# andreicuceu/vega

Measured on AMD Instinct MI355X. Metric: model+chi2 evals/sec (Lya auto+cross), higher is better.
Workload: dtype f64

## Files before the change

### vega_amd/csrc/vegamx.hip

```cpp
#include "vmx_device.h"
#include "vmx_fit.h"
#include "vmx_ensemble.h"
#include "vmx_nested.h"
#include "vmx_smc.h"

#include <atomic>
#include <cmath>
#include <chrono>
#include <thread>
#include <algorithm>
#include <cstdio>
#include <cstdlib>
#include <cstring>
#include <map>
#include <mutex>
#include <queue>
#include <utility>
#include <string>
#include <vector>

#ifndef VMX_MAX_LANES
#define VMX_MAX_LANES 2
#endif

// ... 624 lines not shown
    std::vector<hipEvent_t> ev_join;
    bool finalized = false;
    std::vector<vmx_engine*> lanes;
    int n_lanes = 1;
    int64_t lane_calls = 0;
    hipStream_t last_stream = nullptr;
    const int32_t* call_mock = nullptr;
    FitWorkspace* fitws = nullptr;
    EnsWorkspace* ensws = nullptr;
    NsWorkspace* nsws = nullptr;
    SmcWorkspace* smcws = nullptr;
    hipEvent_t lane_wait = nullptr;

    int nk = 0, nkp = 0, n_mu = 0;
    int n_rows = 0, n_extra = 0, mu_lo = 0, mu_hi = 0;
    DevBuf<double> node_w, mu_img, mu_img_w;
    std::vector<int32_t> rule_slot; std::vector<double> rule_lo, rule_hi;
    DevBuf<int32_t> d_rule_slot; DevBuf<double> d_rule_lo, d_rule_hi;
    double k_node_max = 0.0; bool mu_nodes_on = true;
    DevBuf<double> k, pklin, delta2, mu, sq1mmu2, lnmu, wl, gk, gk_mom, fv_x, fv_f, xtab;
    std::vector<int32_t> const_slots;
    std::vector<int32_t> const_slots2;
    DevBuf<int32_t> d_const_slots, d_const_slots2, d_xtab_pipe, d_xtab_partner;
    DevBuf<double> xtab_k;
    std::vector<int32_t> xi_static_taps, xi_static_bins;
    DevBuf<int32_t> d_xi_static_taps, d_xi_static_bins;
    DevBuf<unsigned long long> gemm_trace;
    size_t gemm_trace_blocks = 0;
    DevBuf<unsigned long long> pk_trace;
    size_t pk_trace_blocks = 0;
    std::vector<int32_t> w_groups;
    DevBuf<int32_t> d_w_groups;
    bool no_pk_w = false;
    std::vector<Tab2Group> tab2_groups;
    DevBuf<double> xtab_key;
    int n_xtab = 0;
    int const_hint = 0;
    int fv_n = 0;
    struct GkSpec { double rp, rt, mock_rp, mock_rt; };
    std::vector<GkSpec> gk_tables;
    std::vector<double> h_k, h_mu;

    int n_coef = 0, ncp = 0, n_knots = 0;
    DevBuf<double> op;
    bool op_set[VMX_MAX_ELL] = {false, false, false, false};
    bool extrapolate = false;
    double x0[VMX_MAX_ELL] = {0}, h[VMX_MAX_ELL] = {0};

    std::vector<PipeDev> pipes;
    std::vector<double> h_r, h_mu_c, h_z, h_relz, h_lnrelz, h_lnrelz2, h_growth;
    DevBuf<double> cr, cmu, crp, crt, cz, crelz, clnrelz, clnrelz2, cgrowth;
    DevBuf<PipeDev> d_pipes;
    std::vector<PkGroup> pk_groups;
    DevBuf<PkGroup> d_pk_groups;
    std::vector<int32_t> pk_members, pk_poly, pk_static;
    DevBuf<int32_t> d_pk_members, d_pk_poly, d_pk_static, d_pipe_active;
    DevBuf<double> poly_coef, poly_bins;
    int64_t poly_bins_total = 0;
    int n_active = 0;
    bool poly_dirty = true;

    std::vector<ItemHost*> items;
    std::vector<MetalHost*> metals;
    DevBuf<ItemDev> d_items;
    DevBuf<MetalDev> d_metals;
    std::vector<double> h_bb, h_odd, h_odd_op;
// ... 1082 lines not shown
int vmx_add_prior(vmx_engine* e, int32_t slot, double mean, double sigma)
{
    REQUIRE(e && !e->finalized && slot >= 0 && sigma != 0.0, "vmx_add_prior");
    e->prior_slot.push_back(slot); e->prior_mean.push_back(mean); e->prior_sigma.push_back(sigma);
    return 0;
}

static int poly_basis_build(vmx_engine* e);
static int xi_sum_plan(vmx_engine* e);

int vmx_finalize(vmx_engine* e, int32_t n_params, int32_t max_batch)
{
    REQUIRE(e && !e->finalized, "vmx_finalize");
    REQUIRE(n_params > 0 && max_batch > 0, "n_params / max_batch");
    REQUIRE(e->nk > 0 && !e->pipes.empty() && !e->items.empty(), "template, pipelines and items are required");
    REQUIRE(e->items.size() <= 16, "at most 16 correlation items");
    REQUIRE(e->pipes.size() * sizeof(PipeDev) <= 48 * 1024, "too many pipelines for the prologue's descriptor stage");
    for (int i = 0; i < VMX_MAX_ELL; ++i) REQUIRE(e->op_set[i], "all four FFTLog operators are required");
    HIP_OK(hipSetDevice(e->device));
    const int Bm = max_batch;
    e->n_params = n_params; e->max_batch = Bm;
    e->slab_rows = Bm > 1024 ? Bm : 1024;
    e->fact_slab_rows = std::max(1024, std::min(4 * Bm, 8192));
    if (getenv("VMX_NO_GRAPH")) e->use_graphs = false;
    if (getenv("VMX_TRACE_HOST")) e->trace_host = true;
    {
        int cus = 256;
        if (hipDeviceGetAttribute(&cus, hipDeviceAttributeMultiprocessorCount, e->device) != hipSuccess || cus <= 0) { (void)hipGetLastError(); cus = 256; }
        e->quad_blocks = 2 * cus;
    }
    if (getenv("VMX_NO_TAB2")) e->no_tab2 = true;
    if (getenv("VMX_NO_CINV_TAPE")) e->no_cinv_tape = true;
    if (getenv("VMX_NO_PK_W")) e->no_pk_w = true;
    if (getenv("VMX_NO_HOST_REDUCE")) e->no_host_reduce = true;
    if (getenv("VMX_NO_XI_LEAN")) e->xi_lean = false;
    if (getenv("VMX_NO_XI_SUMS")) e->xi_sums = false;

    auto slot_ok = [&](int s) { return s < n_params; };
    for (auto& p : e->pipes) {
        const vmx_pipe_desc& d = p.d;
        const int slots[] = {d.tracer[0].bias_slot, d.tracer[0].bias_eta_slot, d.tracer[0].beta_slot,
                             d.tracer[0].vd_sigma_slot, d.tracer[0].alpha_slot, d.tracer[1].bias_slot,
                             d.tracer[1].bias_eta_slot, d.tracer[1].beta_slot, d.tracer[1].vd_sigma_slot,
                             d.tracer[1].alpha_slot, d.growth_rate_slot, d.bias_gamma_slot, d.bias_prim_slot,
                             d.lambda_uv_slot, d.bias_gamma_e_slot, d.lambda_heii_slot, d.bias_hcd_slot,
                             d.beta_hcd_slot, d.l0_hcd_slot, d.sigma_nl_par_slot, d.sigma_nl_per_slot,
                             d.exp_par_slot, d.exp_per_slot, d.scale_slot[0], d.scale_slot[1], d.drp_slot,
                             d.croom_slot[0], d.croom_slot[1], d.mock_los_slot};
        for (int s : slots) REQUIRE(slot_ok(s), "pipeline slot exceeds n_params");
        for (int i = 0; i < 6; ++i) REQUIRE(slot_ok(d.arinyo_slot[i]), "arinyo slot exceeds n_params");
        for (int i = 0; i < d.n_smooth; ++i)
            REQUIRE(d.smooth_par_slot[i] >= 0 && d.smooth_per_slot[i] >= 0 && slot_ok(d.smooth_par_slot[i]) &&
                    slot_ok(d.smooth_per_slot[i]), "smoothing slot");
        for (int q = 0; q < 2; ++q) {
            const vmx_tracer& t = d.tracer[q];
            const int have = (t.bias_slot >= 0) + (t.bias_eta_slot >= 0) + (t.beta_slot >= 0);
            REQUIRE(have >= 2, "each tracer needs two of (bias, bias_eta, beta)");
            REQUIRE(t.evol_kind == VMX_EVOL_CROOM ? (d.croom_slot[0] >= 0 && d.croom_slot[1] >= 0) : t.alpha_slot >= 0,
                    "bias-evolution slot");
            REQUIRE(d.vd_kind == VMX_VD_NONE || !t.discrete || t.vd_sigma_slot >= 0, "velocity dispersion slot");
        }
        REQUIRE(!d.uvb || (d.bias_gamma_slot >= 0 && d.bias_prim_slot >= 0 && d.lambda_uv_slot >= 0), "UVB slots");
        REQUIRE(!d.heii || (d.bias_gamma_e_slot >= 0 && d.bias_prim_slot >= 0 && d.lambda_heii_slot >= 0), "HeII slots");
        REQUIRE(d.hcd_model == VMX_HCD_NONE || (d.bias_hcd_slot >= 0 && d.beta_hcd_slot >= 0), "HCD slots");
        REQUIRE(d.hcd_model != VMX_HCD_ROGERS || d.l0_hcd_slot >= 0, "L0_hcd slot");
        REQUIRE(d.hcd_model != VMX_HCD_FVOIGT || e->fv_n >= 2, "model-hcd = fvoigt needs vmx_set_fvoigt_table");
// ... 774 lines not shown
            hipLaunchKernelGGL(k_pk_poly, dim3(B, (int)e->pk_poly.size()), dim3(256), 0, e->stream, D, e->d_pk_poly.p, B);
        int tm = tab_mode;
        int n_other = n_groups;
        if (tab_mode >= 2 && e->n_xtab > 0) {
            n_other = n_groups - e->n_xtab;
            const size_t sh1 = std::max<size_t>(2048, (size_t)2 * e->n_mu + 4 * e->n_extra + 256 + 16) * sizeof(double);
            if (sh1 > 64 * 1024) {
                static std::mutex mu;
                static size_t allowed[64] = {};
                std::lock_guard<std::mutex> lock(mu);
                size_t& a = allowed[e->device & 63];
                if (sh1 > a) {
                    HIP_OK(hipFuncSetAttribute((const void*)k_pk_tab2<64, 4, 2>, hipFuncAttributeMaxDynamicSharedMemorySize, (int)sh1));
                    HIP_OK(hipFuncSetAttribute((const void*)k_pk_tab2<64, 4, 1>, hipFuncAttributeMaxDynamicSharedMemorySize, (int)sh1));
                    HIP_OK(hipFuncSetAttribute((const void*)k_pk_tab2<16, 16, 1>, hipFuncAttributeMaxDynamicSharedMemorySize, (int)sh1));
                    a = sh1;
                }
            }
#ifdef VMX_EXP_PRO_TRACE
            D.pk_trace = nullptr;
            if (false) {
#else
            if (getenv("VMX_PK_TRACE")) {
#endif
                e->pk_trace_blocks = (size_t)B * ((e->nk + 7) / 8) * e->tab2_groups.size();
                if (!e->pk_trace.p && e->pk_trace.alloc(4 * (size_t)e->max_batch * ((e->nk + 7) / 8) * e->tab2_groups.size(), true)) return -2;
                D.pk_trace = e->pk_trace.p;
            }
            for (size_t first = 0; first < e->tab2_groups.size(); first += VMX_TAB2_GROUPS) {
                Tab2Args A{};
                const int n = (int)std::min<size_t>(VMX_TAB2_GROUPS, e->tab2_groups.size() - first);
                for (int q = 0; q < n; ++q) A.g[q] = e->tab2_groups[first + q];
                if ((int64_t)B * e->n_xtab >= 24) {
                    if (B >= 64)
                        hipLaunchKernelGGL((k_pk_tab2<64, 4, 2>), dim3((B + 1) / 2, n, (e->nk + 63) / 64), dim3(256), std::max(sh1, (size_t)4096 * sizeof(double)), e->stream, D, A, B);
                    else
                        hipLaunchKernelGGL((k_pk_tab2<64, 4, 1>), dim3(B, n, (e->nk + 63) / 64), dim3(256), sh1, e->stream, D, A, B);
                } else
                    hipLaunchKernelGGL((k_pk_tab2<16, 16, 1>), dim3(B, n, (e->nk + 15) / 16), dim3(256), sh1, e->stream, D, A, B);
            }
        }
        const int n_w = ((int64_t)B * (int)e->w_groups.size() >= 24 && !e->no_pk_w) ? (int)e->w_groups.size() : 0;
        if (n_w > 0) {
            n_other -= n_w;
            tm |= 32;
            const size_t shw = std::max<size_t>((size_t)2 * 6 * 256, (size_t)2 * e->n_mu + 4 * e->n_extra + 16) * sizeof(double);
            if (B >= 64)
                hipLaunchKernelGGL((k_pk_w<2>), dim3((B + 1) / 2, n_w, (e->nk + 63) / 64), dim3(256), shw, e->stream, D, e->d_pk_groups.p, e->d_pk_members.p, e->d_w_groups.p, B);
            else
                hipLaunchKernelGGL((k_pk_w<1>), dim3(B, n_w, (e->nk + 63) / 64), dim3(256), shw, e->stream, D, e->d_pk_groups.p, e->d_pk_members.p, e->d_w_groups.p, B);
        }
        if (n_other == 0) {}
        else {
            bool generic = false;
            for (auto& g : e->pk_groups) if (g.variant == PKV_GENERIC) generic = true;
            const PkGroup* gp = e->d_pk_groups.p;
            const int32_t* mp = e->d_pk_members.p;
#define VMX_LAUNCH_PK(KT, MS)                                                                                        \
            do {                                                                                                     \
                const dim3 grid(B, n_groups, (e->nk + (KT) - 1) / (KT));                                             \
                if (generic) hipLaunchKernelGGL((k_pk_multipoles<KT, MS, 1, true>), grid, dim3(256), shmem, e->stream, D, gp, mp, tm, B, mu_tab_off);   \
                else hipLaunchKernelGGL((k_pk_multipoles<KT, MS, 1, false>), grid, dim3(256), shmem, e->stream, D, gp, mp, tm, B, mu_tab_off);         \
            } while (0)
            if ((int64_t)B * n_groups >= 24) VMX_LAUNCH_PK(64, 4);
            else if ((int64_t)B * n_groups >= 4) VMX_LAUNCH_PK(16, 16);
            else {
                shmem = ((size_t)e->n_rows + 2048 + (size_t)8 * e->n_rows) * sizeof(double);
// ... 2048 lines not shown
```

### vega_amd/csrc/vmx_device.h

```cpp
#pragma once
#include <hip/hip_runtime.h>
#include <stdint.h>
#include "../../include/vegamx.h"
#include "vmx_plan.h"

#define VMX_NS 40
#define VMX_PAD 32
#define VMX_MAX_BB 32
#define VMX_MAX_METALS 64
#define VMX_MAX_QUAD_COEF 64
#define VMX_MAX_GROUP 8
#define VMX_MAX_MARG 16

enum {
    S_BIAS1 = 0, S_BB1, S_BIAS2, S_BB2,
    S_UV_BG, S_UV_BP, S_UV_LAM, S_HE_BG, S_HE_LAM,
    S_HCD_B, S_HCD_BB, S_HCD_L0,
    S_GA, S_GB, S_EA, S_EB,
    S_AQ1, S_AQ2, S_AKV, S_AAV, S_ABV, S_AKP,
    S_VD1, S_VD2,
    S_AP, S_AT, S_DRP, S_EV1A, S_EV1B, S_EV2A, S_EV2B,
    S_RAD_S, S_RAD_A, S_RAD_L, S_RAD_D, S_RAD_IL, S_RAD_ID,
    S_NO_RULE
};

static inline int vmx_pad(int n) { return (n + VMX_PAD - 1) / VMX_PAD * VMX_PAD; }

struct PipeDev {
    vmx_pipe_desc d;
    int32_t n;
    int32_t n_pad;
    int64_t coord_off;
    int64_t xi_off;
    double rp_absmin, rp_absmax, rt_min, rt_max;
    int32_t col;
    int32_t poly_basis;
// ... 184 lines not shown
        const double sp = t[d.smooth_par_slot[i]], st = t[d.smooth_per_slot[i]];
        ga += d.smooth_weight[i] * sp * sp; gb += d.smooth_weight[i] * st * st;
    }
    if (d.vd_kind == VMX_VD_GAUSS)
#pragma unroll
        for (int q = 0; q < 2; ++q)
            if (d.tracer[q].discrete) { const double sg = t[d.tracer[q].vd_sigma_slot]; ga += 0.25 * sg * sg; }
}

#define XTAB_ROWS 8
__device__ __forceinline__ double vmx_log(double x);
__device__ void xtab_body(const EngineDev& D, int xtab, int bx, int by, int rows_per_block, const double* t0);

template <bool BYVAL>
__device__ __forceinline__ void prologue_body(const EngineDev& D, int B)
{
    const double* src_all = BYVAL ? (const double*)__builtin_amdgcn_kernarg_segment_ptr() : D.theta_host ? D.theta_host : D.theta;
    if (D.xtab_block0 > 0 && (int)blockIdx.x >= D.xtab_block0) {
        const int rows_per_block = XTAB_ROWS * (256 / PRO_T);
        const int nbx = (D.nkp + PRO_T - 1) / PRO_T, nby = (D.n_rows + rows_per_block - 1) / rows_per_block;
        const int q = (int)blockIdx.x - D.xtab_block0;
        xtab_body(D, q / (nbx * nby), q % nbx, (q / nbx) % nby, rows_per_block, src_all);
        return;
    }
#ifdef VMX_EXP_PRO_TRACE
#define PRO_STAMP(I) do { if (threadIdx.x == 0 && D.pk_trace) D.pk_trace[8 * blockIdx.x + (I)] = wall_clock64(); } while (0)
#else
#define PRO_STAMP(I) do {} while (0)
#endif
    PRO_STAMP(0);
    const int n_chunk = (B + PRO_T - 1) / PRO_T;
    const int slot = (int)blockIdx.x / n_chunk, b_first = ((int)blockIdx.x % n_chunk) * PRO_T;
    const int b = b_first + (int)threadIdx.x;
    if (blockIdx.x == 0 && threadIdx.x == 0) { D.k_live[0] = 0; D.k_live[1] = 0; }
    const bool half_b = slot >= D.n_pipe && slot < 2 * D.n_pipe, walker_slot = slot == 2 * D.n_pipe;
    const int p = min(half_b ? slot - D.n_pipe : slot, D.n_pipe - 1);
    const VMX_CAS PipeDev& P = *(const VMX_CAS PipeDev*)(D.pipes + p);
    extern __shared__ double s_dyn[];
    const int n_cs = D.n_const_slots, n_ru = D.n_rule;
    double* s_c0 = s_dyn;
    double* s_cs = s_c0 + n_cs;
    double* s_ru = s_cs + n_cs;
    double* s_theta = s_ru + 3 * n_ru;
    const int t_ld = D.n_params | 1;
    const int rows = min(B, b_first + PRO_T) - b_first;
    {
        if (BYVAL || D.src_host) {
            const int count = rows * D.n_params;
            const double* src = src_all + (size_t)b_first * D.n_params;
            for (int i0 = threadIdx.x; i0 < count; i0 += 4 * PRO_T) {
                double v[4];
#pragma unroll
                for (int u = 0; u < 4; ++u) { const int i = i0 + u * PRO_T; v[u] = i < count ? src[i] : 0.0; }
#pragma unroll
                for (int u = 0; u < 4; ++u) { const int i = i0 + u * PRO_T; if (i < count) s_theta[(i / D.n_params) * t_ld + i % D.n_params] = v[u]; }
            }
        } else {
            const int nd = 2 * D.n_params;
            const char* src = (const char*)(src_all + (size_t)b_first * D.n_params);
            for (int c0 = 0; c0 < nd; c0 += PRO_T)
                if (c0 + (int)threadIdx.x < nd)
                    for (int r = 0; r < rows; ++r)
                        __builtin_amdgcn_global_load_lds((const __attribute__((address_space(1))) void*)(src + ((size_t)r * nd + c0 + threadIdx.x) * 4),
                                                         (__attribute__((address_space(3))) void*)((char*)(s_theta + r * t_ld) + c0 * 4), 4, 0, 0);
        }
        if (walker_slot)
            for (int i = threadIdx.x; i < n_cs; i += PRO_T) { const int q = D.const_slots[i]; s_cs[i] = (double)q; s_c0[i] = src_all[q]; }
// ... 874 lines not shown
        s_red[(half * 4 + 2) * 256 + threadIdx.x] = (39.375 * m[2] - 33.75 * m[1] + 3.375 * m[0]) * inv_nmu;
        s_red[(half * 4 + 3) * 256 + threadIdx.x] = (187.6875 * m[3] - 255.9375 * m[2] + 85.3125 * m[1] - 4.0625 * m[0]) * inv_nmu;
    }
    __syncthreads();
    if (bad && valid && walker_ok) atomicOr(&D.status[b], VMX_STATUS_ARINYO);

    if (lt < KT && valid && walker_ok) {
        double damp = 1.0;
        if (d.damping_scale > 0.0) damp = exp(-d.damping_scale * d.damping_scale * pow(k, (double)d.damping_power) / 2.0);
        const size_t ncols = (size_t)B * D.n_active;
        for (int half = 0; half < (T.paired ? 2 : 1); ++half) {
            const int pipe = half ? pp : p;
            const int kind = D.pipes[pipe].d.pk_lin_kind;
            const double pk = damp * ((D.pk_direct && kind == VMX_PKLIN_SMOOTH) ? D.pk_direct[(size_t)b * D.nkp + i]
                                                                                 : D.pklin[(size_t)kind * D.nkp + i]);
            const size_t col = (size_t)D.pipes[pipe].col * B + b;
            for (int e = 0; e < D.n_ell; ++e) {
                double sum = 0.0;
                for (int qq = 0; qq < MS; ++qq) sum += s_red[(half * 4 + e) * 256 + (wb * MS + qq) * KT + kk];
                D.pl[((size_t)e * ncols + col) * D.nkp + i] = pk * sum;
            }
        }
    }
}

struct Tab2Group { int32_t pipe, partner, xtab, cross, kind_s, kind_q, col_s, col_q, uvb, heii, lya1, lya2, damping_power, pad;
                   double damping_scale; };
#define VMX_TAB2_GROUPS 8
struct Tab2Args { Tab2Group g[VMX_TAB2_GROUPS]; };

#ifndef VMX_TAB2_PF
#define VMX_TAB2_PF 4
#endif
template <int KT, int MS, int NW, bool CROSS, int MODE = 0>
__device__ __forceinline__ void pk_tab2_body(const EngineDev& D, const Tab2Group& G, int B)
{
    extern __shared__ double smem[];
    constexpr int NT = KT * MS;
    double* s_red = smem;
    v2d* s_mu24 = (v2d*)smem;
    v4d* s_node = (v4d*)(smem + 2 * D.n_mu);
    const int p = G.pipe, pp = G.partner, xt = G.xtab;
    constexpr bool cross = CROSS;
    const int tile = blockIdx.z;
    const unsigned long long t_start = D.pk_trace ? wall_clock64() : 0ull;
    const int kk = threadIdx.x % KT;
    const int ms = (KT == 64) ? __builtin_amdgcn_readfirstlane(threadIdx.x / KT) : (int)(threadIdx.x / KT);
    const int i = tile * KT + kk;
    const bool valid = i < D.nk;
    const int ic = valid ? i : D.nk - 1;
    const int n_mu = D.n_mu;
    const double inv_nmu = 1.0 / (double)n_mu;
    {
        const unsigned total = (2u * (unsigned)n_mu + 4u * (unsigned)D.n_extra) * 8u;
        const char* img = (const char*)D.mu_img;
        const unsigned wave_off = (threadIdx.x >> 6) * 1024u, lane_off = (threadIdx.x & 63) * 16u;
        for (unsigned c = 0; c < total; c += (unsigned)NT * 16u) {
            const unsigned off = c + wave_off;
            if (off + lane_off < total)
                __builtin_amdgcn_global_load_lds((const __attribute__((address_space(1))) void*)(img + off + lane_off),
                                                 (__attribute__((address_space(3))) void*)((char*)smem + off), 16, 0, 0);
        }
    }
    const double* kx = D.xtab_k + (size_t)xt * 4 * D.nkp + ic;
    const double e_max = kx[3 * D.nkp];
    const double bad_flag = kx[2 * D.nkp];
    const double k = D.k[ic], k2 = k * k;
    bool ok[NW];
    double raw[NW][14];
#pragma unroll
    for (int w = 0; w < NW; ++w) {
        int b = blockIdx.x * NW + w;
        ok[w] = b < B;
        if (!ok[w]) b = B - 1;
        const double* sc = D.scal + ((size_t)b * D.n_pipe + p) * VMX_NS;
        raw[w][0] = sc[S_BIAS1]; raw[w][1] = sc[S_BIAS2]; raw[w][2] = sc[S_BB1]; raw[w][3] = sc[S_BB2];
        raw[w][4] = sc[S_HCD_B]; raw[w][5] = sc[S_HCD_BB]; raw[w][6] = sc[S_HCD_L0]; raw[w][7] = sc[S_VD2]; raw[w][8] = sc[S_NO_RULE];
        raw[w][9] = G.uvb ? sc[S_UV_LAM] : 0.0; raw[w][10] = G.uvb ? sc[S_UV_BG] : 0.0; raw[w][11] = (G.uvb || G.heii) ? sc[S_UV_BP] : 0.0;
        raw[w][12] = G.heii ? sc[S_HE_LAM] : 0.0; raw[w][13] = G.heii ? sc[S_HE_BG] : 0.0;
    }
    double* s_x = smem + 2 * (size_t)n_mu + 4 * (size_t)D.n_extra;
    int* s_vote = (int*)(s_x + 2 * NW * KT);
    if (G.uvb || G.heii) {
#pragma unroll
        for (int role = 0; role < 2 * NW; ++role) {
            if (role % MS != ms) continue;
            const int term = role / NW, wsel = role % NW;
            const double lam = term ? raw[wsel][12] : raw[wsel][9], bg = term ? raw[wsel][13] : raw[wsel][10], bp = raw[wsel][11];
            double v = 0.0;
            if (term ? G.heii : G.uvb) { const double x = k * lam; const double W = atan(x) / x; v = bg * W / (1.0 + bp * W); }
            s_x[(size_t)role * KT + kk] = v;
        }
    }
    {
        const unsigned long long live_v = __ballot(!(e_max < VMX_PK_DEAD));
        const unsigned long long rule_v = __ballot(k <= D.k_node_max || e_max < VMX_PK_NEGLIGIBLE), all_v = __ballot(true);
        if ((threadIdx.x & 63) == 0) {
            s_vote[2 * (threadIdx.x >> 6)] = live_v != 0ull;
            s_vote[2 * (threadIdx.x >> 6) + 1] = rule_v == all_v;
        }
    }
    asm volatile("s_waitcnt vmcnt(0)" ::: "memory");
    __syncthreads();
    bool live_block = false, rule_ok = true;
#pragma unroll
    for (int wv = 0; wv < NT / 64; ++wv) { live_block = live_block || s_vote[2 * wv] != 0; rule_ok = rule_ok && s_vote[2 * wv + 1] != 0; }
    if (!live_block) {
        if (threadIdx.x >= KT || !valid) return;
        const size_t ncols = (size_t)B * D.n_active;
        for (int w = 0; w < NW; ++w) {
            const int b = blockIdx.x * NW + w;
            if (b >= B) continue;
            for (int half = 0; half < 2; ++half)
                for (int e = 0; e < D.n_ell; ++e)
                    D.pl[((size_t)e * ncols + (size_t)(half ? G.col_q : G.col_s) * B + b) * D.nkp + i] = 0.0;
        }
        return;
    }
    const double dmu = (double)MS * inv_nmu;
    const bool bad = bad_flag != 0.0;
    double c01[NW], c11[NW], c02[NW], c12[NW], hb[NW], hbb[NW], fk[NW], Fq[NW], k2vd2[NW];
    bool in_box = true;
#pragma unroll
    for (int w = 0; w < NW; ++w) {
        c01[w] = raw[w][0]; c02[w] = raw[w][1]; c11[w] = raw[w][2]; c12[w] = raw[w][3];
        hb[w] = raw[w][4]; hbb[w] = raw[w][5];
        fk[w] = -raw[w][6] * k;
        Fq[w] = vmx_exp(fk[w] * dmu);
        k2vd2[w] = k2 * raw[w][7];
        const bool inside = raw[w][8] == 0.0;
        in_box = in_box && inside;
        if (MODE == 1) ok[w] = ok[w] && inside;
        if (MODE == 2) ok[w] = ok[w] && !inside;
    }
    if (MODE == 1) in_box = true;
    if (MODE == 2) in_box = false;
    if (threadIdx.x == 0) atomicMax(D.k_live, min((tile + 1) * KT, D.nk));
    const bool node_mode = D.n_extra > 0 && in_box && rule_ok;
    if (node_mode && threadIdx.x == 0) atomicMax(D.k_live + 1, min((tile + 1) * KT, D.nk));
    const int lo_end = node_mode ? D.mu_lo : n_mu, hi_beg = node_mode ? n_mu - D.mu_hi : n_mu;
    if (G.uvb || G.heii) {
#pragma unroll
        for (int w = 0; w < NW; ++w) {
            double add = 0.0;
// ... 81 lines not shown
                for (int w = 0; w < NW; ++w) F[w] = vmx_exp(fk[w] * nd.x);                                            \
                VMX_TAB2_NODE(nd.y, nd.z, true, g, h)                                                                 \
            }
            int jj = ms;
            for (int it = 0; it < steps / VMX_TAB2_PF; ++it, jj += VMX_TAB2_PF * MS) {
#pragma unroll
                for (int u = 0; u < VMX_TAB2_PF; ++u) VMX_TAB2_XSTEP(gw[u], hw[u], jj + u * MS)
            }
#pragma unroll
            for (int u = 0; u < VMX_TAB2_PF - 1; ++u)
                if (u < steps % VMX_TAB2_PF) VMX_TAB2_XSTEP(gw[u], hw[u], jj + u * MS)
#undef VMX_TAB2_XSTEP
        }
#undef VMX_TAB2_NODE
    }

#ifdef VMX_EXP_PK_PHASE
    const unsigned long long t_loop = D.pk_trace ? wall_clock64() : 0ull;
#endif
    __syncthreads();
#pragma unroll
    for (int w = 0; w < NW; ++w)
#pragma unroll
        for (int half = 0; half < 2; ++half) {
            const double* m = half ? q[w] : s[w];
            double* r = s_red + (size_t)w * 8 * NT + (half * 4) * NT + threadIdx.x;
            r[0] = m[0] * inv_nmu;
            r[NT] = (7.5 * m[1] - 2.5 * m[0]) * inv_nmu;
            r[2 * NT] = (39.375 * m[2] - 33.75 * m[1] + 3.375 * m[0]) * inv_nmu;
            r[3 * NT] = (187.6875 * m[3] - 255.9375 * m[2] + 85.3125 * m[1] - 4.0625 * m[0]) * inv_nmu;
        }
    __syncthreads();
    if (D.pk_trace && threadIdx.x == 0) {
        unsigned long long* tr = D.pk_trace + 4 * ((size_t)(blockIdx.z * gridDim.y + blockIdx.y) * gridDim.x + blockIdx.x);
        tr[0] = t_start; tr[1] = wall_clock64();
#ifdef VMX_EXP_PK_PHASE
        tr[2] = t_setup; tr[3] = t_loop;
#else
        tr[2] = __builtin_amdgcn_s_getreg((31 << 11) | 4); tr[3] = __builtin_amdgcn_s_getreg((31 << 11) | 20);
#endif
    }
    if (threadIdx.x >= KT || !valid) return;
    double damp = 1.0;
    if (G.damping_scale > 0.0) damp = exp(-G.damping_scale * G.damping_scale * pow(k, (double)G.damping_power) / 2.0);
    const size_t ncols = (size_t)B * D.n_active;
#pragma unroll
    for (int w = 0; w < NW; ++w) {
        if (!ok[w]) continue;
        const int b = blockIdx.x * NW + w;
        if (bad) atomicOr(&D.status[b], VMX_STATUS_ARINYO);
        for (int half = 0; half < 2; ++half) {
            const int kind = half ? G.kind_q : G.kind_s;
            const double pk = damp * ((D.pk_direct && kind == VMX_PKLIN_SMOOTH) ? D.pk_direct[(size_t)b * D.nkp + i]
                                                                                 : D.pklin[(size_t)kind * D.nkp + i]);
            const size_t col = (size_t)(half ? G.col_q : G.col_s) * B + b;
            for (int e = 0; e < D.n_ell; ++e) {
                double sum = 0.0;
                for (int qq = 0; qq < MS; ++qq) sum += s_red[(size_t)w * 8 * NT + (half * 4 + e) * NT + qq * KT + kk];
                D.pl[((size_t)e * ncols + col) * D.nkp + i] = pk * sum;
            }
        }
    }
}

template <int KT, int MS, int NW>
__device__ __forceinline__ void pk_tab2_mixed(const EngineDev& D, const Tab2Group& G, int B)
{
    if (G.cross) pk_tab2_body<KT, MS, NW, true, 1>(D, G, B); else pk_tab2_body<KT, MS, NW, false, 1>(D, G, B);
    __syncthreads();
    if (G.cross) pk_tab2_body<KT, MS, NW, true, 2>(D, G, B); else pk_tab2_body<KT, MS, NW, false, 2>(D, G, B);
}

#ifndef VMX_TAB2_BLOCKS
#define VMX_TAB2_BLOCKS 4
#define VMX_TAB2_W2 3
#endif
template <int KT, int MS, int NW>
__global__ __launch_bounds__(KT * MS, KT != 64 ? 4 : (NW == 1 ? VMX_TAB2_BLOCKS : VMX_TAB2_W2) * (4 / MS)) void k_pk_tab2(EngineDev D, Tab2Args A, int B)
{
    const Tab2Group& G = A.g[blockIdx.y];
    if constexpr (NW > 1) {
        bool any_in = false, all_in = true;
        for (int w = 0; w < NW; ++w) {
            const int b = min((int)blockIdx.x * NW + w, B - 1);
            const bool inside = D.scal[((size_t)b * D.n_pipe + G.pipe) * VMX_NS + S_NO_RULE] == 0.0;
            any_in = any_in || inside; all_in = all_in && inside;
        }
        if (any_in && !all_in) { pk_tab2_mixed<KT, MS, NW>(D, G, B); return; }
    }
    if (G.cross) pk_tab2_body<KT, MS, NW, true>(D, G, B);
    else pk_tab2_body<KT, MS, NW, false>(D, G, B);
}

__global__ __launch_bounds__(256) void k_pk_extrap(EngineDev D, int B)
{
    const size_t ncols = (size_t)B * D.n_active;
    const int e = (int)(blockIdx.x / ncols);
    const int col = (int)((blockIdx.x % ncols) / B);
    double* row = D.pl + (size_t)blockIdx.x * D.nkp;
    const bool used = e < D.pipes[D.pipe_active[col]].d.n_ell;
    const double f0 = row[0], f1 = row[1], fm = row[D.nk - 2], fn = row[D.nk - 1];
    const double ratio_l = f1 / f0, ratio_r = fn / fm;
    for (int t = threadIdx.x; t < D.pad_l + D.pad_r; t += 256) {
        double v = 0.0;
        if (used) v = t < D.pad_l ? f0 * pow(ratio_l, -(double)(t + 1)) : fn * pow(ratio_r, (double)(t - D.pad_l + 1));
        row[D.nk + t] = v;
    }
}

template <int NW, int MODE>
__device__ __forceinline__ void pk_w_body(const EngineDev& D, const PkGroup* groups, const int32_t* members, const int32_t* wlist, int B)
{
    extern __shared__ double smem[];
    constexpr int KT = 64, MS = 4;
    double* s_red = smem;
    v2d* s_mu24 = (v2d*)smem;
    v4d* s_node = (v4d*)(smem + 2 * D.n_mu);
    const PkGroup& G = groups[wlist[blockIdx.y]];
    const int p = G.pipe;
    const vmx_pipe_desc& d = D.pipes[p].d;
    const int tile = blockIdx.z;
    const int kk = threadIdx.x % KT;
    const int ms = __builtin_amdgcn_readfirstlane(threadIdx.x / KT);
    const int i = tile * KT + kk;
// ... 2026 lines not shown
```

### vega_amd/csrc/vmx_plan.h

```cpp
#pragma once
#include <algorithm>
#include <cmath>
#include <cstdint>
#include <functional>
#include <string>
#include <vector>

struct GemmWork { int32_t prob, mt, nt, kbeg, kend, slab, slot, pad; };

namespace vmx_plan {

struct TapeProblem { int nq, nq_pad; };

inline int tape_row0(int nq, int bm) { const int r = nq % bm; return r % 2 == 0 ? r : 0; }
inline int tape_tile_hi(int nq, int mt, int bm)
{
    const int row0 = tape_row0(nq, bm);
    return row0 > 0 ? row0 + mt * bm : (mt + 1) * bm;
}
inline int tape_tile_stages(const TapeProblem& p, int mt, int bm, int bk) { return std::min((tape_tile_hi(p.nq, mt, bm) + bk - 1) / bk, p.nq_pad / bk); }

struct Tape {
    std::vector<GemmWork> work;
    std::vector<int32_t> queue;
    std::vector<int32_t> nt_off;
    std::vector<int32_t> piece_at;
    int n_blocks = 0, group_size = 1, n_pieces = 0;
    int64_t n_slots = 0;
    double capacity = 0.0;
};

inline Tape plan_quad_tape(const std::vector<TapeProblem>& probs, int tn, int blocks, double entry_stages, double skew,
                           int bm = 64, int bk = 32, bool k_bands = false)
{
    Tape T;
    const int P = std::max(blocks / 8 * 8, 8);
    struct Range { int prob, mt, stages; };
    std::vector<Range> ranges;
    for (size_t q = 0; q < probs.size(); ++q) {
        const int tm = (probs[q].nq + bm - 1) / bm;
        for (int mt = 0; mt < tm; ++mt) ranges.push_back({(int)q, mt, tape_tile_stages(probs[q], mt, bm, bk)});
    }
    std::stable_sort(ranges.begin(), ranges.end(), [](const Range& a, const Range& b) { return a.stages > b.stages; });
// ... 254 lines not shown
```

Before: 921,900.

## Add persistent work-queue kernel for tabulated P(k) with cross groups first

Replaces the 3D grid launch of the tabulated P(k) kernel with a persistent kernel sized to occupancy. Blocks pull (slot, group, k-tile) entries from an atomic counter, ordering cross-correlation groups first so the heavier work starts early. The mu/node image is staged into LDS once per block instead of once per tile, and the next index is prefetched with double-buffered shared slots. It adds atomic contention and noinline atan/exp helpers to limit register pressure, and risks load imbalance or lower occupancy if the LDS budget check fails.

Result: slower. 815,800 (-11.5%).

```diff
diff --git a/vega_amd/csrc/vegamx.hip b/vega_amd/csrc/vegamx.hip
--- a/vega_amd/csrc/vegamx.hip
+++ b/vega_amd/csrc/vegamx.hip
@@ -680,6 +680,9 @@
     std::vector<int32_t> w_groups;
     DevBuf<int32_t> d_w_groups;
     bool no_pk_w = false;
+    bool no_pk_queue = false;
+    int pk_queue_blocks = -1;
+    size_t pk_queue_lds = 0;
     std::vector<Tab2Group> tab2_groups;
     DevBuf<double> xtab_key;
     int n_xtab = 0;
@@ -1828,6 +1831,7 @@
     if (getenv("VMX_NO_TAB2")) e->no_tab2 = true;
     if (getenv("VMX_NO_CINV_TAPE")) e->no_cinv_tape = true;
     if (getenv("VMX_NO_PK_W")) e->no_pk_w = true;
+    if (getenv("VMX_NO_PK_QUEUE")) e->no_pk_queue = true;
     if (getenv("VMX_NO_HOST_REDUCE")) e->no_host_reduce = true;
     if (getenv("VMX_NO_XI_LEAN")) e->xi_lean = false;
     if (getenv("VMX_NO_XI_SUMS")) e->xi_sums = false;
@@ -2668,7 +2672,29 @@
                 const int n = (int)std::min<size_t>(VMX_TAB2_GROUPS, e->tab2_groups.size() - first);
                 for (int q = 0; q < n; ++q) A.g[q] = e->tab2_groups[first + q];
                 if ((int64_t)B * e->n_xtab >= 24) {
-                    if (B >= 64)
+                    int q_blocks = 0, q_cross = -1;
+                    const size_t shq = ((size_t)2 * e->n_mu + 4 * e->n_extra + 16 + 4096) * sizeof(double);
+                    if (B >= 64 && !e->no_pk_queue && e->tab2_groups.size() <= VMX_TAB2_GROUPS) {
+                        std::vector<int> is_cross;
+                        for (auto& g : e->tab2_groups) is_cross.push_back(g.cross);
+                        q_cross = vmx_plan::pk_queue_cross_first(is_cross);
+                        if (e->pk_queue_blocks < 0 || e->pk_queue_lds != shq) {
+                            int per_cu = 0, cus = 0;
+                            e->pk_queue_blocks = 0; e->pk_queue_lds = shq;
+                            if ((shq + 2047) / 2048 * 2048 * VMX_TAB2_W2 <= 160 * 1024 &&
+                                hipFuncSetAttribute((const void*)k_pk_tab2_queue<64, 4, 2>, hipFuncAttributeMaxDynamicSharedMemorySize, (int)shq) == hipSuccess &&
+                                hipOccupancyMaxActiveBlocksPerMultiprocessor(&per_cu, k_pk_tab2_queue<64, 4, 2>, 256, shq) == hipSuccess &&
+                                hipDeviceGetAttribute(&cus, hipDeviceAttributeMultiprocessorCount, e->device) == hipSuccess &&
+                                per_cu >= VMX_TAB2_W2 && cus > 0)
+                                e->pk_queue_blocks = per_cu * cus;
+                            else (void)hipGetLastError();
+                        }
+                        if (q_cross >= 0) q_blocks = e->pk_queue_blocks;
+                    }
+                    if (q_blocks > 0) {
+                        const int n_entries = vmx_plan::pk_queue_size((B + 1) / 2, n, (e->nk + 63) / 64);
+                        hipLaunchKernelGGL((k_pk_tab2_queue<64, 4, 2>), dim3(std::min(q_blocks, n_entries)), dim3(256), shq, e->stream, D, A, B, n, q_cross);
+                    } else if (B >= 64)
                         hipLaunchKernelGGL((k_pk_tab2<64, 4, 2>), dim3((B + 1) / 2, n, (e->nk + 63) / 64), dim3(256), std::max(sh1, (size_t)4096 * sizeof(double)), e->stream, D, A, B);
                     else
                         hipLaunchKernelGGL((k_pk_tab2<64, 4, 1>), dim3(B, n, (e->nk + 63) / 64), dim3(256), sh1, e->stream, D, A, B);
diff --git a/vega_amd/csrc/vmx_device.h b/vega_amd/csrc/vmx_device.h
--- a/vega_amd/csrc/vmx_device.h
+++ b/vega_amd/csrc/vmx_device.h
@@ -1,7 +1,9 @@
 #pragma once
 #include <hip/hip_runtime.h>
 #include <stdint.h>
+#include <type_traits>
 #include "../../include/vegamx.h"
+#define VMX_PLAN_FN __host__ __device__ inline
 #include "vmx_plan.h"
 
 #define VMX_NS 40
@@ -252,7 +254,7 @@
     const int n_chunk = (B + PRO_T - 1) / PRO_T;
     const int slot = (int)blockIdx.x / n_chunk, b_first = ((int)blockIdx.x % n_chunk) * PRO_T;
     const int b = b_first + (int)threadIdx.x;
-    if (blockIdx.x == 0 && threadIdx.x == 0) { D.k_live[0] = 0; D.k_live[1] = 0; }
+    if (blockIdx.x == 0 && threadIdx.x == 0) { D.k_live[0] = 0; D.k_live[1] = 0; D.k_live[5] = 0; }
     const bool half_b = slot >= D.n_pipe && slot < 2 * D.n_pipe, walker_slot = slot == 2 * D.n_pipe;
     const int p = min(half_b ? slot - D.n_pipe : slot, D.n_pipe - 1);
     const VMX_CAS PipeDev& P = *(const VMX_CAS PipeDev*)(D.pipes + p);
@@ -1193,17 +1195,20 @@
 #ifndef VMX_TAB2_PF
 #define VMX_TAB2_PF 4
 #endif
-template <int KT, int MS, int NW, bool CROSS, int MODE = 0>
-__device__ __forceinline__ void pk_tab2_body(const EngineDev& D, const Tab2Group& G, int B)
+__device__ __attribute__((noinline)) static double pk_tab2_atan(double x) { return atan(x); }
+__device__ __attribute__((noinline)) static double pk_tab2_damping(double scale, int power, double k) { return exp(-scale * scale * pow(k, (double)power) / 2.0); }
+
+template <int KT, int MS, int NW, bool CROSS, int MODE = 0, bool PERSIST = false>
+__device__ __forceinline__ void pk_tab2_body(const EngineDev& D, const Tab2Group& G, int B, const int bx, const int tile,
+                                             const size_t trace_at, const int par = 0, int* s_next = nullptr, const int nxt = 0)
 {
     extern __shared__ double smem[];
     constexpr int NT = KT * MS;
-    double* s_red = smem;
+    double* s_red = PERSIST ? smem + 2 * (size_t)D.n_mu + 4 * (size_t)D.n_extra + 16 : smem;
     v2d* s_mu24 = (v2d*)smem;
     v4d* s_node = (v4d*)(smem + 2 * D.n_mu);
     const int p = G.pipe, pp = G.partner, xt = G.xtab;
     constexpr bool cross = CROSS;
-    const int tile = blockIdx.z;
     const unsigned long long t_start = D.pk_trace ? wall_clock64() : 0ull;
     const int kk = threadIdx.x % KT;
     const int ms = (KT == 64) ? __builtin_amdgcn_readfirstlane(threadIdx.x / KT) : (int)(threadIdx.x / KT);
@@ -1212,7 +1217,7 @@
     const int ic = valid ? i : D.nk - 1;
     const int n_mu = D.n_mu;
     const double inv_nmu = 1.0 / (double)n_mu;
-    {
+    if (!PERSIST) {
         const unsigned total = (2u * (unsigned)n_mu + 4u * (unsigned)D.n_extra) * 8u;
         const char* img = (const char*)D.mu_img;
         const unsigned wave_off = (threadIdx.x >> 6) * 1024u, lane_off = (threadIdx.x & 63) * 16u;
@@ -1231,17 +1236,19 @@
     double raw[NW][14];
 #pragma unroll
     for (int w = 0; w < NW; ++w) {
-        int b = blockIdx.x * NW + w;
+        int b = bx * NW + w;
         ok[w] = b < B;
         if (!ok[w]) b = B - 1;
-        const double* sc = D.scal + ((size_t)b * D.n_pipe + p) * VMX_NS;
+        typedef typename std::conditional<PERSIST, const VMX_CAS double*, const double*>::type scal_ptr;
+        const scal_ptr sc = (scal_ptr)(D.scal + ((size_t)b * D.n_pipe + p) * VMX_NS);
         raw[w][0] = sc[S_BIAS1]; raw[w][1] = sc[S_BIAS2]; raw[w][2] = sc[S_BB1]; raw[w][3] = sc[S_BB2];
         raw[w][4] = sc[S_HCD_B]; raw[w][5] = sc[S_HCD_BB]; raw[w][6] = sc[S_HCD_L0]; raw[w][7] = sc[S_VD2]; raw[w][8] = sc[S_NO_RULE];
         raw[w][9] = G.uvb ? sc[S_UV_LAM] : 0.0; raw[w][10] = G.uvb ? sc[S_UV_BG] : 0.0; raw[w][11] = (G.uvb || G.heii) ? sc[S_UV_BP] : 0.0;
         raw[w][12] = G.heii ? sc[S_HE_LAM] : 0.0; raw[w][13] = G.heii ? sc[S_HE_BG] : 0.0;
     }
-    double* s_x = smem + 2 * (size_t)n_mu + 4 * (size_t)D.n_extra;
-    int* s_vote = (int*)(s_x + 2 * NW * KT);
+    double* s_x = PERSIST ? s_red : smem + 2 * (size_t)n_mu + 4 * (size_t)D.n_extra;
+    int* s_vote = PERSIST ? (int*)(smem + 2 * (size_t)n_mu + 4 * (size_t)D.n_extra) + par * 2 * (NT / 64)
+                          : (int*)(s_x + 2 * NW * KT);
     if (G.uvb || G.heii) {
 #pragma unroll
         for (int role = 0; role < 2 * NW; ++role) {
@@ -1249,7 +1256,7 @@
             const int term = role / NW, wsel = role % NW;
             const double lam = term ? raw[wsel][12] : raw[wsel][9], bg = term ? raw[wsel][13] : raw[wsel][10], bp = raw[wsel][11];
             double v = 0.0;
-            if (term ? G.heii : G.uvb) { const double x = k * lam; const double W = atan(x) / x; v = bg * W / (1.0 + bp * W); }
+            if (term ? G.heii : G.uvb) { const double x = k * lam; const double W = (PERSIST ? pk_tab2_atan(x) : atan(x)) / x; v = bg * W / (1.0 + bp * W); }
             s_x[(size_t)role * KT + kk] = v;
         }
     }
@@ -1261,6 +1268,7 @@
             s_vote[2 * (threadIdx.x >> 6) + 1] = rule_v == all_v;
         }
     }
+    if (PERSIST && s_next && threadIdx.x == 0) *s_next = nxt;
     asm volatile("s_waitcnt vmcnt(0)" ::: "memory");
     __syncthreads();
     bool live_block = false, rule_ok = true;
@@ -1270,7 +1278,7 @@
         if (threadIdx.x >= KT || !valid) return;
         const size_t ncols = (size_t)B * D.n_active;
         for (int w = 0; w < NW; ++w) {
-            const int b = blockIdx.x * NW + w;
+            const int b = bx * NW + w;
             if (b >= B) continue;
             for (int half = 0; half < 2; ++half)
                 for (int e = 0; e < D.n_ell; ++e)
@@ -1418,7 +1426,7 @@
         }
     __syncthreads();
     if (D.pk_trace && threadIdx.x == 0) {
-        unsigned long long* tr = D.pk_trace + 4 * ((size_t)(blockIdx.z * gridDim.y + blockIdx.y) * gridDim.x + blockIdx.x);
+        unsigned long long* tr = D.pk_trace + 4 * trace_at;
         tr[0] = t_start; tr[1] = wall_clock64();
 #ifdef VMX_EXP_PK_PHASE
         tr[2] = t_setup; tr[3] = t_loop;
@@ -1428,12 +1436,14 @@
     }
     if (threadIdx.x >= KT || !valid) return;
     double damp = 1.0;
-    if (G.damping_scale > 0.0) damp = exp(-G.damping_scale * G.damping_scale * pow(k, (double)G.damping_power) / 2.0);
+    if (G.damping_scale > 0.0)
+        damp = PERSIST ? pk_tab2_damping(G.damping_scale, G.damping_power, k)
+                       : exp(-G.damping_scale * G.damping_scale * pow(k, (double)G.damping_power) / 2.0);
     const size_t ncols = (size_t)B * D.n_active;
 #pragma unroll
     for (int w = 0; w < NW; ++w) {
         if (!ok[w]) continue;
-        const int b = blockIdx.x * NW + w;
+        const int b = bx * NW + w;
         if (bad) atomicOr(&D.status[b], VMX_STATUS_ARINYO);
         for (int half = 0; half < 2; ++half) {
             const int kind = half ? G.kind_q : G.kind_s;
@@ -1449,12 +1459,27 @@
     }
 }
 
-template <int KT, int MS, int NW>
-__device__ __forceinline__ void pk_tab2_mixed(const EngineDev& D, const Tab2Group& G, int B)
-{
-    if (G.cross) pk_tab2_body<KT, MS, NW, true, 1>(D, G, B); else pk_tab2_body<KT, MS, NW, false, 1>(D, G, B);
+template <int KT, int MS, int NW, bool PERSIST = false>
+__device__ __forceinline__ void pk_tab2_mixed(const EngineDev& D, const Tab2Group& G, int B, const int bx, const int tile,
+                                              const size_t trace_at, const int par = 0, int* s_next = nullptr, const int nxt = 0)
+{
+    if (G.cross) pk_tab2_body<KT, MS, NW, true, 1, PERSIST>(D, G, B, bx, tile, trace_at, par, s_next, nxt);
+    else pk_tab2_body<KT, MS, NW, false, 1, PERSIST>(D, G, B, bx, tile, trace_at, par, s_next, nxt);
     __syncthreads();
-    if (G.cross) pk_tab2_body<KT, MS, NW, true, 2>(D, G, B); else pk_tab2_body<KT, MS, NW, false, 2>(D, G, B);
+    if (G.cross) pk_tab2_body<KT, MS, NW, true, 2, PERSIST>(D, G, B, bx, tile, trace_at, par);
+    else pk_tab2_body<KT, MS, NW, false, 2, PERSIST>(D, G, B, bx, tile, trace_at, par);
+}
+
+template <int NW>
+__device__ __forceinline__ bool pk_tab2_walkers_disagree(const EngineDev& D, const Tab2Group& G, int B, const int bx)
+{
+    bool any_in = false, all_in = true;
+    for (int w = 0; w < NW; ++w) {
+        const int b = min(bx * NW + w, B - 1);
+        const bool inside = D.scal[((size_t)b * D.n_pipe + G.pipe) * VMX_NS + S_NO_RULE] == 0.0;
+        any_in = any_in || inside; all_in = all_in && inside;
+    }
+    return any_in && !all_in;
 }
 
 #ifndef VMX_TAB2_BLOCKS
@@ -1465,17 +1490,49 @@
 __global__ __launch_bounds__(KT * MS, KT != 64 ? 4 : (NW == 1 ? VMX_TAB2_BLOCKS : VMX_TAB2_W2) * (4 / MS)) void k_pk_tab2(EngineDev D, Tab2Args A, int B)
 {
     const Tab2Group& G = A.g[blockIdx.y];
+    const int bx = blockIdx.x, tile = blockIdx.z;
+    const size_t trace_at = (size_t)(blockIdx.z * gridDim.y + blockIdx.y) * gridDim.x + blockIdx.x;
     if constexpr (NW > 1) {
-        bool any_in = false, all_in = true;
-        for (int w = 0; w < NW; ++w) {
-            const int b = min((int)blockIdx.x * NW + w, B - 1);
-            const bool inside = D.scal[((size_t)b * D.n_pipe + G.pipe) * VMX_NS + S_NO_RULE] == 0.0;
-            any_in = any_in || inside; all_in = all_in && inside;
-        }
-        if (any_in && !all_in) { pk_tab2_mixed<KT, MS, NW>(D, G, B); return; }
-    }
-    if (G.cross) pk_tab2_body<KT, MS, NW, true>(D, G, B);
-    else pk_tab2_body<KT, MS, NW, false>(D, G, B);
+        if (pk_tab2_walkers_disagree<NW>(D, G, B, bx)) { pk_tab2_mixed<KT, MS, NW>(D, G, B, bx, tile, trace_at); return; }
+    }
+    if (G.cross) pk_tab2_body<KT, MS, NW, true>(D, G, B, bx, tile, trace_at);
+    else pk_tab2_body<KT, MS, NW, false>(D, G, B, bx, tile, trace_at);
+}
+
+template <int KT, int MS, int NW>
+__global__ __launch_bounds__(KT * MS, VMX_TAB2_W2 * (4 / MS)) void k_pk_tab2_queue(EngineDev D, Tab2Args A, int B, int n_groups, int n_cross)
+{
+    extern __shared__ double smem[];
+    constexpr int NT = KT * MS;
+    int* s_next = (int*)(smem + 2 * (size_t)D.n_mu + 4 * (size_t)D.n_extra) + 4 * (NT / 64);
+    {
+        const unsigned total = (2u * (unsigned)D.n_mu + 4u * (unsigned)D.n_extra) * 8u;
+        const char* img = (const char*)D.mu_img;
+        const unsigned wave_off = (threadIdx.x >> 6) * 1024u, lane_off = (threadIdx.x & 63) * 16u;
+        for (unsigned c = 0; c < total; c += (unsigned)NT * 16u) {
+            const unsigned off = c + wave_off;
+            if (off + lane_off < total)
+                __builtin_amdgcn_global_load_lds((const __attribute__((address_space(1))) void*)(img + off + lane_off),
+                                                 (__attribute__((address_space(3))) void*)((char*)smem + off), 16, 0, 0);
+        }
+    }
+    const int n_slots = (B + NW - 1) / NW, n_tiles = (D.nk + KT - 1) / KT;
+    const int n_entries = vmx_plan::pk_queue_size(n_slots, n_groups, n_tiles);
+    if (threadIdx.x == 0) s_next[0] = atomicAdd(D.k_live + 5, 1);
+    __syncthreads();
+    int cur = __builtin_amdgcn_readfirstlane(s_next[0]), par = 1;
+    while (cur < n_entries) {
+        int nxt = 0;
+        if (threadIdx.x == 0) nxt = atomicAdd(D.k_live + 5, 1);
+        const vmx_plan::PkEntry en = vmx_plan::pk_queue_entry(cur, n_slots, n_cross, n_groups, n_tiles);
+        const Tab2Group& G = A.g[en.group];
+        if (pk_tab2_walkers_disagree<NW>(D, G, B, en.slot)) pk_tab2_mixed<KT, MS, NW, true>(D, G, B, en.slot, en.tile, (size_t)cur, par, s_next + par, nxt);
+        else if (G.cross) pk_tab2_body<KT, MS, NW, true, 0, true>(D, G, B, en.slot, en.tile, (size_t)cur, par, s_next + par, nxt);
+        else pk_tab2_body<KT, MS, NW, false, 0, true>(D, G, B, en.slot, en.tile, (size_t)cur, par, s_next + par, nxt);
+        cur = __builtin_amdgcn_readfirstlane(s_next[par]);
+        par ^= 1;
+        __syncthreads();
+    }
 }
 
 __global__ __launch_bounds__(256) void k_pk_extrap(EngineDev D, int B)
diff --git a/vega_amd/csrc/vmx_plan.h b/vega_amd/csrc/vmx_plan.h
--- a/vega_amd/csrc/vmx_plan.h
+++ b/vega_amd/csrc/vmx_plan.h
@@ -8,7 +8,46 @@
 
 struct GemmWork { int32_t prob, mt, nt, kbeg, kend, slab, slot, pad; };
 
+#ifndef VMX_PLAN_FN
+#define VMX_PLAN_FN inline
+#endif
+
 namespace vmx_plan {
+
+struct PkEntry { int32_t slot, group, tile; };
+VMX_PLAN_FN int pk_queue_size(int n_slots, int n_groups, int n_tiles) { return n_slots * n_groups * n_tiles; }
+VMX_PLAN_FN PkEntry pk_queue_entry(int idx, int n_slots, int n_cross, int n_groups, int n_tiles)
+{
+    const int cross_entries = n_slots * n_cross * n_tiles;
+    int r = idx, g0 = 0, ng = n_cross;
+    if (idx >= cross_entries) { r -= cross_entries; g0 = n_cross; ng = n_groups - n_cross; }
+    const int per_tile = n_slots * ng;
+    PkEntry e;
+    e.tile = r / per_tile;
+    r -= e.tile * per_tile;
+    e.group = g0 + r / n_slots;
+    e.slot = r - (r / n_slots) * n_slots;
+    return e;
+}
+inline int pk_queue_cross_first(const std::vector<int>& group_is_cross)
+{
+    int n_cross = 0;
+    while (n_cross < (int)group_is_cross.size() && group_is_cross[n_cross]) ++n_cross;
+    for (size_t g = n_cross; g < group_is_cross.size(); ++g) if (group_is_cross[g]) return -1;
+    return n_cross;
+}
+inline std::vector<PkEntry> plan_pk_queue(int B, int nw, const std::vector<int>& group_is_cross, int nk, int kt)
+{
+    std::vector<PkEntry> q;
+    const int n_cross = pk_queue_cross_first(group_is_cross), n_groups = (int)group_is_cross.size();
+    if (B <= 0 || nw <= 0 || nk <= 0 || kt <= 0 || n_groups == 0 || n_cross < 0) return q;
+    const int n_slots = (B + nw - 1) / nw, n_tiles = (nk + kt - 1) / kt;
+    if ((int64_t)n_slots * n_groups * n_tiles > (int64_t)1 << 30) return q;
+    const int n = pk_queue_size(n_slots, n_groups, n_tiles);
+    q.reserve((size_t)n);
+    for (int idx = 0; idx < n; ++idx) q.push_back(pk_queue_entry(idx, n_slots, n_cross, n_groups, n_tiles));
+    return q;
+}
 
 struct TapeProblem { int nq, nq_pad; };
 
```
